# octaviogarcia/RaytracingOneWeekend

Hardware: AMD Instinct MI355X
Metric: Msamples/s (W×H×spp/s) + achieved HBM GB/s, 1080p@512spp traced scene (higher is better)
Workload: dtype f32; 1 GPU; C1 S-traced 1920x1080, 10496 spp timed (128 spp/step), depth 50; width=1920, height=1080, max_depth=50, parallelism=tile1, gather=RCCL send/recv (om_gather_frame), rccl_library=/usr/local/lib/python3.10/dist-packages/torch/lib/librccl.so, kernel=auto, pipeline=auto, tail_bounce=default, streams=2

## Files before the change

include/ottomarcher.h:

```cpp
#ifndef OTTOMARCHER_H
#define OTTOMARCHER_H

#include <stdint.h>
#include <stddef.h>

#ifdef __cplusplus
extern "C" {
#endif

#define OM_ABI_VERSION 2

typedef int32_t om_status;
#define OM_OK 0
#define OM_ERR_INVALID (-1)
#define OM_ERR_DEVICE (-2)
#define OM_ERR_STATE (-3)
#define OM_ERR_UNSUPPORTED (-4)
#define OM_ERR_NOMEM (-5)

enum { OM_LAMBERTIAN = 0, OM_METAL = 1, OM_DIELECTRIC = 2 };
typedef struct om_material {
    float albedo[3];
    float fuzz;
    float ior;
// ... 147 lines not shown
om_status om_occluded_rays(om_ctx* ctx, const om_query_params* q, const om_ray* rays,
                           const om_ray_window* windows, uint32_t n, uint8_t* occluded);
om_status om_hit_rays_windows_device(om_ctx* ctx, const om_query_params* q, const om_ray* dev_rays,
                                     const om_ray_window* dev_windows, uint32_t n, om_hit* dev_hits, void* stream);
om_status om_hit_rays_windows(om_ctx* ctx, const om_query_params* q, const om_ray* rays,
                              const om_ray_window* windows, uint32_t n, om_hit* hits);
#define OM_QUERY_BLOCK 512
uint32_t om_query_max_grid(om_ctx* ctx);
om_status om_host_register(void* p, size_t bytes);
om_status om_host_unregister(void* p);
om_status om_render_device(om_ctx* ctx, const om_camera* cam, const om_render_params* p, om_pixel_stats* dev_stats,
                           void* stream);
om_status om_render_device_pixels(om_ctx* ctx, const om_camera* cam, const om_render_params* p, om_pixel_stats* dev_stats,
                                  const uint32_t* dev_pixels, uint32_t n_pixels, void* stream);
om_status om_get_counters(om_ctx* ctx, om_counters* out);
om_status om_reset_counters(om_ctx* ctx, void* stream);
const volatile uint64_t* om_progress(om_ctx* ctx);
om_status om_reset_progress(om_ctx* ctx);
om_status om_set_counting(om_ctx* ctx, int32_t enable);
enum { OM_PIPELINE_MEGAKERNEL = 0, OM_PIPELINE_WAVEFRONT = 1, OM_PIPELINE_AUTO = 2 };
om_status om_set_pipeline(om_ctx* ctx, int32_t pipeline);
om_status om_set_tail_bounce(om_ctx* ctx, uint32_t bounce);

om_status om_set_streams(om_ctx* ctx, uint32_t streams);

om_status om_set_adaptive_batches(om_ctx* ctx, uint32_t batches, uint32_t paths_log2);

enum { OM_PRIMARY_LISTS_OFF = 0, OM_PRIMARY_LISTS_AUTO = 1, OM_PRIMARY_LISTS_ON = 2 };
om_status om_set_primary_lists(om_ctx* ctx, int32_t mode);

enum {
    OM_KT_BOUNCE0 = 0,
    OM_KT_BOUNCE = 1,
    OM_KT_TAIL = 2,
    OM_KT_ACCUMULATE = 3,
    OM_KT_MEGAKERNEL = 4,
    OM_KT_BOUNCE_SPAN = 5,
    OM_KT_N = 6
};
typedef struct om_kernel_times {
    uint64_t launches[OM_KT_N];
    double ms[OM_KT_N];
} om_kernel_times;
om_status om_set_timing(om_ctx* ctx, int32_t mode);
om_status om_get_kernel_times(om_ctx* ctx, om_kernel_times* out);

// ... 57 lines not shown
```

raytracingoneweekend_amd/_lib.py:

```python
import ctypes as C
import os

import numpy as np

_HERE = os.path.dirname(os.path.abspath(__file__))
LIB_PATH = os.environ.get("OM_LIB") or os.path.join(_HERE, "libottomarcher.so")

OM_OK = 0
OM_ERR_INVALID, OM_ERR_DEVICE, OM_ERR_STATE, OM_ERR_UNSUPPORTED, OM_ERR_NOMEM = -1, -2, -3, -4, -5
OM_LAMBERTIAN, OM_METAL, OM_DIELECTRIC = 0, 1, 2
OM_KERNEL_AUTO, OM_KERNEL_BRUTE, OM_KERNEL_CULLED, OM_KERNEL_BVH, OM_KERNEL_SBVH, OM_KERNEL_BVH2, OM_KERNEL_BVH4 = \
    0, 1, 2, 3, 4, 5, 6
OM_KERNEL_BVH2W = 7
KERNELS = {"auto": OM_KERNEL_AUTO, "brute": OM_KERNEL_BRUTE, "culled": OM_KERNEL_CULLED, "bvh": OM_KERNEL_BVH,
           "sbvh": OM_KERNEL_SBVH, "bvh2": OM_KERNEL_BVH2, "bvh4": OM_KERNEL_BVH4, "bvh2w": OM_KERNEL_BVH2W}
TREE_REGIMES = ("none", "lds", "l2", "wide", "fallback_bvh")
OM_PIPELINE_MEGAKERNEL, OM_PIPELINE_WAVEFRONT, OM_PIPELINE_AUTO = 0, 1, 2
PIPELINES = {"megakernel": OM_PIPELINE_MEGAKERNEL, "wavefront": OM_PIPELINE_WAVEFRONT, "auto": OM_PIPELINE_AUTO}

F3 = C.c_float * 3
F16 = C.c_float * 16


class om_material(C.Structure):
# ... 65 lines not shown
KT_CLASSES = ("bounce0", "bounce", "tail", "accumulate", "megakernel", "bounce_span")
VIEWS = ("normal", "samples", "sample_blur", "depth", "depth_blur", "ids", "id_blur")


class om_kernel_times(C.Structure):
    _fields_ = [("launches", C.c_uint64 * 6), ("ms", C.c_double * 6)]


PIXEL_STATS_DTYPE = np.dtype([("bloom", "<u8"), ("sum", "<f4", (3,)), ("n", "<u4"), ("avg_depth", "<f4"),
                              ("bad_avgs", "<u4"), ("color", "u1", (3,)), ("flags", "u1"), ("reserved", "<u4")])
assert PIXEL_STATS_DTYPE.itemsize == 40

EXPORTS = [
    "om_abi_version", "om_build_id", "om_material_lambertian", "om_material_metal", "om_material_metal_fuzz", "om_material_dielectric",
    "om_mat4_identity", "om_mat4_translate", "om_mat4_scale", "om_mat4_rotate", "om_mat4_mul",
    "om_mat4_fast_homogenous_inverse", "om_camera_new", "om_world_create", "om_world_destroy", "om_world_clear",
    "om_world_add_sphere", "om_world_add_sphere_radius", "om_world_add_cube", "om_world_add_cube_length",
    "om_world_add_triangle", "om_world_add_parallelogram", "om_world_add_triangle_basis",
    "om_world_add_parallelogram_basis", "om_world_add_plane", "om_world_add_marched_sphere",
    "om_world_add_marched_box", "om_world_add_marched_torus", "om_world_add_marched_sdf", "om_world_marched_sdf_count", "om_world_counts", "om_world_export",
    "om_world_random_scene", "om_world_basic_scene", "om_world_marched_scene", "om_create", "om_destroy",
    "om_last_error", "om_upload_world", "om_set_kernel", "om_render", "om_render_device",
    "om_render_device_pixels", "om_get_counters", "om_reset_counters", "om_set_counting", "om_set_pipeline",
    "om_set_tail_bounce", "om_set_streams", "om_set_adaptive_batches", "om_set_timing", "om_get_kernel_times", "om_display_device", "om_display",
    "om_write_bmp", "om_write_ppm", "om_set_primary_lists",
    "om_shard_capacity", "om_shard_pixels", "om_shard_assemble_host", "om_comm_unique_id", "om_comm_init_rank",
    "om_comm_destroy", "om_comm_info", "om_render_shard", "om_gather_frame", "om_scatter_frame", "om_multi_create",
    "om_multi_destroy", "om_multi_transport", "om_multi_ctx", "om_multi_upload_world", "om_multi_render",
    "om_multi_last_error", "om_progress", "om_reset_progress", "om_host_register", "om_host_unregister",
    "om_multi_render_host", "om_multi_gather", "om_multi_reset", "om_rccl_library",
    "om_hit_rays_device", "om_hit_rays", "om_world_object_material", "om_query_max_grid",
    "om_occluded_rays_device", "om_occluded_rays", "om_hit_rays_windows_device", "om_hit_rays_windows",
    "om_world_add_triangles", "om_world_tree_info", "om_get_tree_info",
]
OM_COMM_ID_BYTES = 128
OM_TRANSPORT_RCCL, OM_TRANSPORT_LOCAL = 0, 1


class OmError(RuntimeError):
    pass


def _share_hip_runtime_with_torch():
    try:
        import torch
    except Exception:
        pass
# ... 40 lines not shown
        "om_world_add_marched_sphere": (st, [vp, fp, C.c_float, mp]),
        "om_world_add_marched_box": (st, [vp, fp, fp, mp]),
        "om_world_add_marched_torus": (st, [vp, fp, fp, mp]),
        "om_world_add_marched_sdf": (st, [vp, fp, vp, C.c_uint32, mp]),
        "om_world_marched_sdf_count": (st, [vp, C.POINTER(C.c_uint32)]),
        "om_world_counts": (st, [vp, C.POINTER(C.c_uint32)]),
        "om_world_export": (st, [vp, C.c_int32, C.c_uint32, fp, C.c_uint32]),
        "om_world_random_scene": (st, [vp, C.c_uint64, C.c_uint32, C.c_int32]),
        "om_world_basic_scene": (st, [vp]),
        "om_world_marched_scene": (st, [vp]),
        "om_create": (st, [C.c_int32, C.POINTER(vp)]),
        "om_destroy": (None, [vp]),
        "om_last_error": (C.c_char_p, [vp]),
        "om_upload_world": (st, [vp, vp]),
        "om_set_kernel": (st, [vp, C.c_int32]),
        "om_render": (st, [vp, C.POINTER(om_camera), C.POINTER(om_render_params), vp, C.POINTER(om_counters)]),
        "om_render_device": (st, [vp, C.POINTER(om_camera), C.POINTER(om_render_params), vp, vp]),
        "om_render_device_pixels": (st, [vp, C.POINTER(om_camera), C.POINTER(om_render_params), vp, vp, C.c_uint32, vp]),
        "om_get_counters": (st, [vp, C.POINTER(om_counters)]),
        "om_reset_counters": (st, [vp, vp]),
        "om_set_counting": (st, [vp, C.c_int32]),
        "om_set_pipeline": (st, [vp, C.c_int32]),
        "om_set_tail_bounce": (st, [vp, C.c_uint32]),
        "om_set_streams": (st, [vp, C.c_uint32]),
        "om_set_adaptive_batches": (st, [vp, C.c_uint32, C.c_uint32]),
        "om_set_timing": (st, [vp, C.c_int32]),
        "om_get_kernel_times": (st, [vp, C.POINTER(om_kernel_times)]),
        "om_display_device": (st, [vp, vp, C.c_uint32, C.c_uint32, C.c_int32, vp, vp]),
        "om_display": (st, [vp, vp, C.c_uint32, C.c_uint32, C.c_int32, vp]),
        "om_write_bmp": (st, [C.c_char_p, vp, C.c_uint32, C.c_uint32]),
        "om_write_ppm": (st, [C.c_char_p, vp, C.c_uint32, C.c_uint32]),
        "om_set_primary_lists": (st, [vp, C.c_int32]),
        "om_shard_capacity": (C.c_uint32, [C.c_uint32, C.c_uint32, C.c_uint32]),
        "om_shard_pixels": (st, [C.c_uint32, C.c_uint32, C.c_uint32, C.c_uint32, vp, C.c_uint32, C.POINTER(C.c_uint32)]),
        "om_shard_assemble_host": (st, [C.c_uint32, C.c_uint32, C.c_uint32, C.POINTER(vp), vp]),
        "om_comm_unique_id": (st, [vp]),
        "om_comm_init_rank": (st, [vp, C.c_uint32, C.c_uint32, vp, C.POINTER(vp)]),
        "om_comm_destroy": (None, [vp]),
        "om_render_shard": (st, [vp, C.POINTER(om_camera), C.POINTER(om_render_params), vp, vp]),
        "om_gather_frame": (st, [vp, vp, C.c_uint32, C.c_uint32, vp, vp]),
        "om_scatter_frame": (st, [vp, vp, C.c_uint32, C.c_uint32, vp, vp]),
        "om_multi_create": (st, [C.POINTER(C.c_int32), C.c_uint32, C.POINTER(vp)]),
        "om_multi_destroy": (None, [vp]),
        "om_multi_transport": (C.c_int32, [vp]),
        "om_multi_ctx": (vp, [vp, C.c_uint32]),
        "om_multi_upload_world": (st, [vp, vp]),
# ... 59 lines not shown
```

raytracingoneweekend_amd/csrc/om_render.hip:

```cpp
#include <hip/hip_runtime.h>

#include <algorithm>
#include <cmath>
#include <cstring>
#include <mutex>
#include <new>
#include <string>
#include <vector>

#include "../../include/ottomarcher.h"
#include "om_device.h"
#include "om_layout.h"
#include "om_display.h"
#include "om_tiles.h"
#include "om_wavefront.h"
#include "om_world.h"
#include "om_internal.h"

using namespace omd;

static_assert(sizeof(om_pixel_stats) == 40, "om_pixel_stats layout");
static_assert(sizeof(om_ray) == 24 && sizeof(om_hit) == 32 && sizeof(om_query_params) == 16, "query record layouts");
static_assert(sizeof(om_ray_window) == 8, "query window layout");
static_assert(OM_QUERY_BLOCK == 512, "OM_QUERY_BLOCK is the wavefront workgroup size");
// ... 201 lines not shown
    void* p = nullptr;
    size_t n = 0;
    void release() { if (p) (void)hipFree(p); p = nullptr; n = 0; }
};

}

struct om_ctx {
    int device = 0;
    hipStream_t stream = nullptr;
    std::string err;
    std::vector<DevBuf> scene_bufs;
    OmSceneDev scene{};
    bool have_world = false;
    om_tree_info tree_info{};
    int kernel = OM_KERNEL_AUTO;
    DevBuf counters, stats, pixels, view_scratch, view_rgb;
    struct JitterTable { uint64_t seed; uint32_t spp; DevBuf buf; };
    std::vector<JitterTable> jitters;
    hipStream_t last_stream = nullptr;
    bool count_work = true;
    int pipeline = OM_PIPELINE_AUTO;
    uint32_t tail_bounce = 0;
    uint32_t wf_streams = 2;
    uint32_t ad_batches = 0, ad_paths_log2 = 0;
    std::vector<float> srec_box;
    uint64_t world_gen = 0;
    int primary_lists = OM_PRIMARY_LISTS_AUTO;
    DevBuf tile_off, tile_idx, tile_tnear;
    bool tiles_valid = false, tiles_use = false;
    om_camera tiles_cam{};
    uint32_t tiles_w = 0, tiles_h = 0;
    uint64_t tiles_gen = 0;
    double tiles_avg = 0.0;
    omw::Timer timer;
    omw::Buffers wf;
    unsigned long long* progress_host = nullptr;
    DevBuf frame_list;
    DevBuf query_rays, query_hits;
    DevBuf query_windows, query_occ;
    uint32_t frame_w = 0, frame_h = 0;
    ~om_ctx() {
        for (auto& b : scene_bufs) b.release();
        for (auto& j : jitters) j.buf.release();
        counters.release(); stats.release(); pixels.release(); frame_list.release();
        query_rays.release(); query_hits.release();
// ... 187 lines not shown
    P.progress = c->progress_host ? 1u : 0u;
    uint64_t threads;
    if (dev_pixels) {
        P.n_pixels = n_pixels;
        threads = n_pixels;
    } else {
        const uint64_t tiles = (uint64_t)P.tiles_x * ((p->height + 7u) / 8u);
        P.n_pixels = p->width * p->height;
        threads = tiles * 64u;
    }
    if (threads == 0) return OM_OK;
    int pipeline = c->pipeline;
    if (pipeline == OM_PIPELINE_AUTO) pipeline = OM_PIPELINE_WAVEFRONT;
    int mode = c->kernel;
    if (mode == OM_KERNEL_AUTO) mode = OM_KERNEL_BVH2;
    if (pipeline == OM_PIPELINE_WAVEFRONT) {
        omw::Launch L;
        L.S = c->scene; L.C = C; L.P = P;
        L.jitter = jitter;
        L.stats = dev_stats;
        L.counters = (unsigned long long*)c->counters.p;
        L.count = c->count_work;
        L.tail_bounce = c->tail_bounce;
        L.streams = c->wf_streams;
        L.ad_batches = c->ad_batches; L.ad_paths_log2 = c->ad_paths_log2;
        L.timer = &c->timer;
        L.tile_off = nullptr; L.tile_idx = nullptr; L.tile_tnear = nullptr;
        L.progress_host = c->progress_host;
        if ((mode == OM_KERNEL_BVH2 && c->scene.n_b2nodes) || (mode == OM_KERNEL_BVH2W && c->scene.n_b2wnodes)) {
            if ((s = ensure_tile_lists(c, cam, p->width, p->height, stream)) != OM_OK) return s;
            if (c->tiles_use) {
                L.tile_off = (const uint32_t*)c->tile_off.p; L.tile_idx = (const uint16_t*)c->tile_idx.p;
                L.tile_tnear = (const float*)c->tile_tnear.p;
            }
        }
        L.trace_mode = wf_trace_mode(mode);
        if (dev_pixels) {
            L.pixels = dev_pixels; L.n_pixels = n_pixels; L.stats_by_pixel = false;
        } else {
            if (c->frame_w != p->width || c->frame_h != p->height || !c->frame_list.p) {
                std::vector<uint32_t> lst;
                lst.reserve((size_t)p->width * p->height);
                const uint32_t tx = (p->width + 7u) / 8u, ty = (p->height + 7u) / 8u;
                for (uint32_t t = 0; t < tx * ty; ++t)
                    for (uint32_t l = 0; l < 64u; ++l) {
                        const uint32_t px = (t % tx) * 8u + (l & 7u), py = (t / tx) * 8u + (l >> 3);
// ... 308 lines not shown

om_status om_set_pipeline(om_ctx* c, int32_t pipeline) {
    if (!c) return set_err(nullptr, OM_ERR_INVALID, "null ctx");
    if (pipeline != OM_PIPELINE_MEGAKERNEL && pipeline != OM_PIPELINE_WAVEFRONT && pipeline != OM_PIPELINE_AUTO)
        return set_err(c, OM_ERR_INVALID, "om_set_pipeline: unknown pipeline");
    c->pipeline = pipeline;
    return OM_OK;
}

om_status om_set_primary_lists(om_ctx* c, int32_t mode) {
    if (!c) return set_err(nullptr, OM_ERR_INVALID, "null ctx");
    if (mode < OM_PRIMARY_LISTS_OFF || mode > OM_PRIMARY_LISTS_ON)
        return set_err(c, OM_ERR_INVALID, "om_set_primary_lists: unknown mode");
    c->primary_lists = mode;
    return OM_OK;
}

om_status om_set_tail_bounce(om_ctx* c, uint32_t bounce) {
    if (!c) return set_err(nullptr, OM_ERR_INVALID, "null ctx");
    c->tail_bounce = bounce;
    return OM_OK;
}

om_status om_set_streams(om_ctx* c, uint32_t streams) {
    if (!c) return set_err(nullptr, OM_ERR_INVALID, "null ctx");
    if (streams < 1 || streams > (uint32_t)omw::kMaxSets) return set_err(c, OM_ERR_INVALID, "om_set_streams: streams must be 1..4");
    c->wf_streams = streams;
    return OM_OK;
}

om_status om_set_adaptive_batches(om_ctx* c, uint32_t batches, uint32_t paths_log2) {
    if (!c) return set_err(nullptr, OM_ERR_INVALID, "null ctx");
    if (batches > 64u || paths_log2 > 27u)
        return set_err(c, OM_ERR_INVALID, "om_set_adaptive_batches: batches <= 64, paths_log2 <= 27");
    c->ad_batches = batches; c->ad_paths_log2 = paths_log2;
    return OM_OK;
}

om_status om_set_timing(om_ctx* c, int32_t mode) {
    if (!c) return set_err(nullptr, OM_ERR_INVALID, "null ctx");
    if (mode < 0 || mode > 2) return set_err(c, OM_ERR_INVALID, "om_set_timing: mode must be 0, 1 or 2");
    OM_HIP(c, hipSetDevice(c->device));
    for (size_t i = 0; c->timer.on() && i < c->timer.cls.size(); ++i)
        if (c->timer.cls[i] >= 0) OM_HIP(c, hipEventSynchronize(c->timer.ev[2 * i + 1]));
    c->timer.mode = mode;
    c->timer.clear();
// ... 120 lines not shown
```

raytracingoneweekend_amd/csrc/om_tuning.h:

```cpp
#pragma once

#ifndef OM_WF_BLOCK
#define OM_WF_BLOCK 512
#endif
#ifndef OM_WF_WAVES
#define OM_WF_WAVES 8
#endif
#ifndef OM_WF_TAIL_SPB
#define OM_WF_TAIL_SPB 2
#endif
#ifndef OM_WF_TAIL_WGS_PER_CU
#define OM_WF_TAIL_WGS_PER_CU 1
#endif
#ifndef OM_WF_MAX_PATHS_LOG2
#define OM_WF_MAX_PATHS_LOG2 27
#endif
#ifndef OM_WF_BATCH_SPP
#define OM_WF_BATCH_SPP 16
#endif
#ifndef OM_WF_MIN_PATHS_LOG2
#define OM_WF_MIN_PATHS_LOG2 25
#endif
#ifndef OM_WF_HYB_BYTES
#define OM_WF_HYB_BYTES 16384
#endif
#ifndef OM_WF_HYBW_BYTES
#define OM_WF_HYBW_BYTES 0
#endif
#ifndef OM_WF_HYB4_BYTES
#define OM_WF_HYB4_BYTES 0
#endif
#ifndef OM_WF_REFILL
#define OM_WF_REFILL 16
#endif
#ifndef OM_WF_TAIL_SHADE
// ... 45 lines not shown
```

raytracingoneweekend_amd/csrc/om_wavefront.h:

```cpp
#pragma once
#include <hip/hip_runtime.h>

#include <cstdint>
#include <string>
#include <vector>

#include "../../include/ottomarcher.h"
#include "om_layout.h"

namespace omw {

struct QueueSet {
    float4* q[2][3] = {{nullptr, nullptr, nullptr}, {nullptr, nullptr, nullptr}};
    uint4* qr[2] = {nullptr, nullptr};
    float4* res = nullptr;
    uint32_t* res_id = nullptr;
    uint32_t* counts = nullptr;
    float2* hit = nullptr;
    void release();
};

constexpr int kMaxSets = 4;
struct Buffers {
    uint64_t cap = 0;
    uint32_t counts_n = 0;
    int nsets = 0;
    QueueSet set[kMaxSets];
    uint32_t* n0 = nullptr;
    uint64_t n0_cap = 0;
    hipStream_t side[kMaxSets] = {};
    std::vector<hipEvent_t> ev;
    void release();
};
// ... 20 lines not shown
    void end(int i, int c, hipStream_t st, uint32_t launches = 1) {
        if (!on() || i < 0) return;
        (void)hipEventRecord(ev[2 * i + 1], st);
        cls[i] = c;
        nl[i] = launches;
    }
    void clear() { cls.clear(); nl.clear(); }
    void release() { for (auto e : ev) (void)hipEventDestroy(e); ev.clear(); clear(); }
};

struct Launch {
    OmSceneDev S;
    OmCamDev C;
    OmParamsDev P;
    const float2* jitter;
    om_pixel_stats* stats;
    const uint32_t* pixels;
    uint32_t n_pixels;
    bool stats_by_pixel;
    unsigned long long* counters;
    bool count;
    int trace_mode;
    uint32_t tail_bounce;
    uint32_t streams;
    uint32_t ad_batches;
    uint32_t ad_paths_log2;
    Timer* timer;
    const uint32_t* tile_off;
    const uint16_t* tile_idx;
    const float* tile_tnear;
    unsigned long long* progress_host;
};

hipError_t render(Buffers& B, const Launch& L, hipStream_t stream, std::string& err);

struct Query {
    OmSceneDev S;
    float tmin, tmax;
    uint32_t march_steps;
    const om_ray* rays;
    const om_ray_window* windows = nullptr;
    om_hit* hits = nullptr;
    uint8_t* occluded = nullptr;
    uint32_t n;
    unsigned long long* counters;
    bool count;
// ... 8 lines not shown
```

raytracingoneweekend_amd/csrc/om_wavefront.hip:

```cpp
#include "om_wavefront.h"

#include <algorithm>
#include <type_traits>

#include "om_device.h"
#include "om_trace.h"
#include "om_tuning.h"

using namespace omd;

namespace omw {

void QueueSet::release() {
    for (int a = 0; a < 2; ++a) {
        for (int b = 0; b < 3; ++b) { if (q[a][b]) (void)hipFree(q[a][b]); q[a][b] = nullptr; }
        if (qr[a]) (void)hipFree(qr[a]); qr[a] = nullptr;
    }
    if (res) (void)hipFree(res);
    if (res_id) (void)hipFree(res_id);
    if (counts) (void)hipFree(counts);
    if (hit) (void)hipFree(hit);
    res = nullptr; res_id = nullptr; counts = nullptr; hit = nullptr;
}

// ... 306 lines not shown
        s = (v & 0x7FFFFFFFu) + R.done + s_local;
        live = s < P.spp_total && !(v >> 31);
    } else {
        const om_pixel_stats& ps = R.stats[R.by_pixel ? pixel : k];
        s = ps.n + s_local;
        live = s < P.spp_total && !(P.adaptive && (ps.flags & 1u));
    }
    if (!live) {
        res_id[i] = kNoSample;
        return false;
    }
    p.g = path_rng(P.skey, pixel, s);
    const uint32_t line = pixel / P.width;
    gen_camera_ray(R.C, P, R.jitter, (float)(pixel - P.width * line), (float)line, s, p.g, p.o, p.d);
    p.cur = f3(1.0f, 1.0f, 1.0f); p.depthf = 0.0f; p.first_id = 0u; p.seg = 0u; p.slot = (uint32_t)i;
    return true;
}

template <int TR, bool COUNT, bool MARCH, bool FIRST, bool HIT = false, bool USER = MARCH>
__global__ __launch_bounds__(kBlk) OM_WAVES_ATTR void k_bounce(OmSceneDev S, OmParamsDev P, Seg G, Gen R, Queue in,
                                                 const uint32_t* __restrict__ count_in, Queue out,
                                                 uint32_t* __restrict__ count_out, float4* __restrict__ res,
                                                 uint32_t* __restrict__ res_id, unsigned long long* __restrict__ counters,
                                                 const float2* __restrict__ hitbuf, uint32_t* __restrict__ tail_next) {
    const uint64_t seg0 = (uint64_t)blockIdx.x * G.segcap;
    uint32_t n, stride = R.n_pixels;
    uint64_t first0 = seg0;
    if (FIRST) {
        if (tail_next && blockIdx.x == 0 && threadIdx.x == 0) *tail_next = 0u;
        uint64_t paths = (uint64_t)R.n_pixels * R.batch;
        if (R.ad.list) {
            const AdPlan pl = uniform_load(R.ad.plan);
            stride = pl.c;
            paths = (uint64_t)pl.c * ad_batch(pl.c, pl.done, R.ad.j, R.ad.A);
            first0 = (uint64_t)blockIdx.x * seg_capacity(paths, G.nseg);
            n = first0 < paths ? (uint32_t)std::min<uint64_t>(seg_capacity(paths, G.nseg), paths - first0) : 0u;
        } else {
            n = seg0 < paths ? (uint32_t)std::min<uint64_t>(G.segcap, paths - seg0) : 0u;
        }
    } else {
        n = count_in[blockIdx.x];
    }
    if (n == 0) {
        if (threadIdx.x == 0) count_out[blockIdx.x] = 0u;
        return;
    }
    __shared__ uint32_t q_next, q_out;
    if (threadIdx.x == 0) { q_next = kBlk / 64u; q_out = 0u; }
    __syncthreads();
    const Tracer T = HIT ? Tracer{} : stage_scene<TR>(S);
    const uint32_t depth_cap = P.max_depth > 1u ? P.max_depth : 1u;
    WorkT<COUNT, false, tr_bary(TR)> w;
    uint32_t segs = 0;
    const uint32_t lane = __lane_id();
    for (uint32_t chunk = __builtin_amdgcn_readfirstlane(threadIdx.x >> 6); chunk * 64u < n;) {
        const uint32_t jj = chunk * 64u + lane;
        bool keep = false;
        Path p;
        uint32_t p_pixel = 0;
        if (jj < n) {
            const uint64_t i = seg0 + jj;
            bool live = true;
            if (FIRST) {
                live = gen_path(P, R, stride, first0 + jj, p, p_pixel, res_id);
            } else {
                load_ray(in, i, p);
                load_rest(in, i, p);
            }
            if (live) {
                float closest;
                int best;
                if (HIT) {
                    const float2 h = hitbuf[i];
                    closest = h.x; best = __float_as_int(h.y);
                } else if (FIRST && (tr_base(TR) == TR_BVH2_LDS || tr_base(TR) == TR_BVH2_GLOBAL || tr_base(TR) == TR_BVH2_WIDE) && R.tile_off) {
                    const uint32_t line = p_pixel / P.width;
                    const uint32_t tile = (p_pixel - line * P.width) / 8u + (line / 8u) * P.tiles_x;
                    closest = P.tmax;
                    const uint32_t t0 = __builtin_amdgcn_readfirstlane(tile);
                    if (__ballot(tile != t0) == 0)
                        best = traced_tiles<true>(S, R.tile_off, R.tile_idx, t0, p.o, p.d, P.tmin, closest, w, R.tile_tnear);
                    else
                        best = traced_tiles(S, R.tile_off, R.tile_idx, tile, p.o, p.d, P.tmin, closest, w);
                    if (MARCH) {
                        float tm;
                        const int mg = march(S, p.o, p.d, P.tmin, P.tmax, closest, P.march_steps, tm, w);
                        if (mg >= 0) { best = mg; closest = tm; }
                    }
                } else {
                    best = trace<TR, MARCH>(S, P, T, p.o, p.d, closest, w);
                }
                keep = shade_path<MARCH, USER>(S, P, depth_cap, p, closest, best, res, res_id);
                if (COUNT) segs++;
            }
        }
        const uint64_t m = __ballot(keep);
        uint32_t obase = 0u, nc = 0u;
        if (lane == 0) {
            obase = m ? atomicAdd(&q_out, (uint32_t)__popcll(m)) : 0u;
            nc = atomicAdd(&q_next, 1u);
        }
        obase = __builtin_amdgcn_readfirstlane(obase);
        chunk = __builtin_amdgcn_readfirstlane(nc);
        if (keep) store_path(out, seg0 + obase + (uint32_t)__popcll(m & ((1ull << lane) - 1ull)), p);
    }
    __syncthreads();
    if (threadIdx.x == 0) count_out[blockIdx.x] = q_out;
    if (COUNT) {
        flush_counter(counters, OMC_SEGMENTS, segs);
        flush_counter(counters, OMC_PRIM_TESTS, w.prim);
        flush_counter(counters, OMC_PRE_TESTS, w.pre);
        flush_counter(counters, OMC_MARCH, w.march);
    }
}

template <bool COUNT>
__global__ __launch_bounds__(kBlk) OM_WAVES_ATTR void k_raygen(OmParamsDev P, Seg G, Gen R, Queue out,
                                                 uint32_t* __restrict__ count_out, uint32_t* __restrict__ res_id) {
    const uint64_t seg0 = (uint64_t)blockIdx.x * G.segcap;
    uint64_t paths = (uint64_t)R.n_pixels * R.batch, first0 = seg0;
    uint32_t n, stride = R.n_pixels;
    if (R.ad.list) {
        const AdPlan pl = uniform_load(R.ad.plan);
        stride = pl.c;
        paths = (uint64_t)pl.c * ad_batch(pl.c, pl.done, R.ad.j, R.ad.A);
        first0 = (uint64_t)blockIdx.x * seg_capacity(paths, G.nseg);
        n = first0 < paths ? (uint32_t)std::min<uint64_t>(seg_capacity(paths, G.nseg), paths - first0) : 0u;
    } else {
        n = seg0 < paths ? (uint32_t)std::min<uint64_t>(G.segcap, paths - seg0) : 0u;
    }
// ... 68 lines not shown
                                                const uint32_t* __restrict__ count_in, float2* __restrict__ hit,
                                                unsigned long long* __restrict__ counters) {
    const uint32_t n = count_in[blockIdx.x];
    if (n == 0) return;
    const uint64_t seg0 = (uint64_t)blockIdx.x * G.segcap;
    __shared__ uint32_t next;
    if (threadIdx.x == 0) next = kBlk;
    __syncthreads();
    const Tracer T = stage_scene<TR>(S);
    WorkT<COUNT, false, tr_bary(TR)> w;
    if constexpr (VIEW == MV_EXACT_C2_LDS) {
        __shared__ MarchedC2Lds::Block mblock;
        march_lanes<TR, COUNT>(S, P, T, MarchedC2Lds(S, &mblock), in, seg0, n, next, hit, w);
    } else {
        march_lanes<TR, COUNT>(S, P, T, MarchedArrays(S), in, seg0, n, next, hit, w);
    }
    if (COUNT) {
        flush_counter(counters, OMC_PRIM_TESTS, w.prim);
        flush_counter(counters, OMC_PRE_TESTS, w.pre);
        flush_counter(counters, OMC_MARCH, w.march);
    }
}

struct TailSrc {
    const Queue& in;
    const uint32_t* pre;
    uint32_t s0, ns, segcap;
    __device__ __forceinline__ bool load(uint32_t idx, Path& p) const {
        uint32_t lo = 0, hi = ns;
        while (hi - lo > 1u) {
            const uint32_t mid = (lo + hi) >> 1;
            if (pre[mid] <= idx) lo = mid; else hi = mid;
        }
        const uint64_t i = (uint64_t)(s0 + lo) * segcap + (idx - pre[lo]);
        load_ray(in, i, p);
        load_rest(in, i, p);
        return true;
    }
};
template <int TR, bool COUNT, class M, class Src, class Wk>
__device__ __forceinline__ uint32_t tail_march_lanes(const OmSceneDev& S, const OmParamsDev& P, const Tracer& T, const M& m,
                                                     const Src& src, uint32_t total, uint32_t& next,
                                                     float4* __restrict__ res, uint32_t* __restrict__ res_id, Wk& w) {
    const uint32_t lane = __lane_id();
    const uint32_t depth_cap = P.max_depth > 1u ? P.max_depth : 1u;
    uint32_t idx = threadIdx.x, segs = 0, iters = 0;
    bool have = idx < total, dry = !have, marching = false, act = false;
    __shared__ uint32_t rest[9][kBlk];
    Path p;
    float t = 0.0f, closest = 0.0f;
    int best = -1;
    auto park = [&]() {
        const uint32_t i = threadIdx.x;
        rest[0][i] = __float_as_uint(p.cur.x); rest[1][i] = __float_as_uint(p.cur.y); rest[2][i] = __float_as_uint(p.cur.z);
        rest[3][i] = __float_as_uint(p.depthf); rest[4][i] = p.first_id; rest[5][i] = p.seg; rest[6][i] = p.slot;
        rest[7][i] = p.g.s; rest[8][i] = p.g.k;
    };
// ... 47 lines not shown
}

template <int TR, bool COUNT, int VIEW = MV_ARRAYS, uint32_t SPB = kTailSpb>
__global__ __launch_bounds__(kBlk) __attribute__((amdgpu_waves_per_eu(OM_WF_TAIL_MARCH_WAVES, OM_WF_TAIL_MARCH_WAVES)))
void k_tail_march(OmSceneDev S, OmParamsDev P, Seg G, Queue in,
                                               const uint32_t* __restrict__ count_in, float4* __restrict__ res,
                                               uint32_t* __restrict__ res_id, unsigned long long* __restrict__ counters) {
    __shared__ uint32_t pre[SPB + 1];
    __shared__ uint32_t next;
    const uint32_t s0 = blockIdx.x * SPB;
    if (threadIdx.x == 0) {
        uint32_t acc = 0;
        for (uint32_t k = 0; k < SPB; ++k) {
            pre[k] = acc;
            acc += s0 + k < G.nseg ? count_in[s0 + k] : 0u;
        }
        pre[SPB] = acc;
        next = kBlk;
    }
    __syncthreads();
    const uint32_t total = pre[SPB];
    if (total == 0) return;
    const Tracer T = stage_scene<TR>(S);
    const TailSrc src{in, pre, s0, SPB, G.segcap};
    WorkT<COUNT, false, tr_bary(TR)> w;
    uint32_t segs = 0;
    if constexpr (VIEW == MV_EXACT_C2_LDS) {
        __shared__ MarchedC2Lds::Block mblock;
        segs = tail_march_lanes<TR, COUNT>(S, P, T, MarchedC2Lds(S, &mblock), src, total, next, res, res_id, w);
    } else {
        segs = tail_march_lanes<TR, COUNT>(S, P, T, MarchedArrays(S), src, total, next, res, res_id, w);
    }
    if (COUNT) {
        flush_counter(counters, OMC_SEGMENTS, segs);
        flush_counter(counters, OMC_PRIM_TESTS, w.prim);
        flush_counter(counters, OMC_PRE_TESTS, w.pre);
        flush_counter(counters, OMC_MARCH, w.march);
    }
}

template <int TR, bool COUNT>
__global__ __launch_bounds__(kBlk) OM_WAVES_ATTR
void k_tail(OmSceneDev S, OmParamsDev P, Seg G, Queue in, const uint32_t* __restrict__ count_in, uint32_t pre_off,
            uint32_t* __restrict__ next, float4* __restrict__ res, uint32_t* __restrict__ res_id,
            unsigned long long* __restrict__ counters) {
    uint32_t* pre = (uint32_t*)wf_lds + pre_off / 4u;
    __shared__ uint32_t wave_sum[kWaves];
    const uint32_t lane = __lane_id(), wave = threadIdx.x >> 6;
    const uint32_t per = (G.nseg + kBlk - 1u) / kBlk;
    const uint32_t c0 = threadIdx.x * per, c1 = c0 + per < G.nseg ? c0 + per : G.nseg;
    uint32_t mine = 0;
    for (uint32_t k = c0; k < c1; ++k) mine += count_in[k];
    uint32_t incl = mine;
#pragma unroll
    for (int off = 1; off < 64; off <<= 1) {
        const uint32_t v = __shfl_up(incl, off, 64);
        if (lane >= (uint32_t)off) incl += v;
    }
    if (lane == 63u) wave_sum[wave] = incl;
    __syncthreads();
    uint32_t acc = incl - mine, total = 0;
#pragma unroll
    for (uint32_t k = 0; k < kWaves; ++k) {
        const uint32_t v = wave_sum[k];
        if (k < wave) acc += v;
        total += v;
    }
    if (total == 0) return;
    for (uint32_t k = c0; k < c1; ++k) { pre[k] = acc; acc += count_in[k]; }
    if (threadIdx.x == 0) pre[G.nseg] = total;
    __syncthreads();
    const Tracer T = stage_scene<TR>(S);
    const uint32_t depth_cap = P.max_depth > 1u ? P.max_depth : 1u;
    const TailSrc src{in, pre, 0u, G.nseg, G.segcap};
    WorkT<COUNT, false, tr_bary(TR)> w;
    uint32_t segs = 0;
    const uint32_t lanes = gridDim.x * kBlk;
    const uint32_t round = (wave + kWaves - blockIdx.x % kWaves) % kWaves;
    uint32_t idx = (round * gridDim.x + blockIdx.x) * 64u + lane;
    bool have = idx < total;
    bool more = total > lanes;
    Path p;
    if (have) src.load(idx, p);
    for (;;) {
        if (have) {
            float closest;
            const int best = trace<TR, false>(S, P, T, p.o, p.d, closest, w);
            if (COUNT) segs++;
            have = shade_path<false>(S, P, depth_cap, p, closest, best, res, res_id);
        }
        if (more) {
            const uint64_t want = __ballot(!have);
            if (want) {
                const uint32_t nw = (uint32_t)__popcll(want);
                uint32_t base = 0u;
                if (lane == 0) base = atomicAdd(next, nw);
                base = lanes + __builtin_amdgcn_readfirstlane(base);
// ... 289 lines not shown
            QueueSet& S = B.set[k];
            if (S.counts) (void)hipFree(S.counts);
            S.counts = nullptr;
            if ((e = hipMalloc(&S.counts, (size_t)counts_n * sizeof(uint32_t))) != hipSuccess) return e;
        }
        B.counts_n = counts_n;
    }
    return hipSuccess;
}

Queue queue(QueueSet& B, int k) { return Queue{B.q[k][0], B.q[k][1], B.q[k][2], B.qr[k]}; }

inline uint32_t tail_pre_off(uint32_t lds) { return (lds + 15u) & ~15u; }
inline uint32_t tail_lds(uint32_t lds, uint32_t nseg) { return tail_pre_off(lds) + (nseg + 1u) * 4u; }

template <int TR, bool COUNT, bool MARCH>
uint32_t run_batch(QueueSet& B, const Launch& L, hipStream_t st, Seg G, const Gen& R, uint32_t depth_cap,
                   uint32_t tail_at, uint32_t lds, uint32_t tail_grid) {
    Timer& tm = *L.timer;
    const bool each = tm.mode == 1;
    uint32_t launches = 0;
    const bool exact = MARCH && L.S.n_msdf == 0u && MarchedC2Lds::matches(L.S.n_msph, L.S.n_mbox, L.S.n_mtor);
    uint32_t* const tail_next = B.counts + (size_t)(depth_cap + 1u) * G.nseg;
    auto tail = [&](const Queue& in, const uint32_t* cin) {
        const int ti = each ? tm.begin(st) : -1;
        if constexpr (MARCH) {
            const uint32_t grid = (G.nseg + kTailSpb - 1u) / kTailSpb;
            if (exact && exact_view_built<TR>())
                hipLaunchKernelGGL((k_tail_march<TR, COUNT, exact_view_built<TR>() ? MV_EXACT_C2_LDS : MV_ARRAYS>), dim3(grid),
                                   dim3(kBlk), lds, st, L.S, L.P, G, in, cin, B.res, B.res_id, L.counters);
            else
                hipLaunchKernelGGL((k_tail_march<TR, COUNT>), dim3(grid), dim3(kBlk), lds, st, L.S, L.P, G, in, cin,
                                   B.res, B.res_id, L.counters);
        } else {
            hipLaunchKernelGGL((k_tail<TR, COUNT>), dim3(tail_grid), dim3(kBlk), tail_lds(lds, G.nseg), st, L.S, L.P, G, in, cin,
                               tail_pre_off(lds), tail_next, B.res, B.res_id, L.counters);
        }
        tm.end(ti, OM_KT_TAIL, st);
        return launches + 1u;
    };
    if constexpr (MARCH) {
        {
            const int ti = each ? tm.begin(st) : -1;
            hipLaunchKernelGGL((k_raygen<COUNT>), dim3(G.nseg), dim3(kBlk), 0, st, L.P, G, R, queue(B, 0), B.counts, B.res_id);
            tm.end(ti, OM_KT_BOUNCE0, st);
            ++launches;
        }
        for (uint32_t bounce = 0; bounce < depth_cap; ++bounce) {
            const Queue in = queue(B, bounce & 1u), out = queue(B, (bounce + 1u) & 1u);
            const uint32_t* cin = B.counts + (size_t)bounce * G.nseg;
            if (bounce >= tail_at) return tail(in, cin);
            uint32_t* cout = B.counts + (size_t)(bounce + 1u) * G.nseg;
            const int kc = bounce == 0 ? OM_KT_BOUNCE0 : OM_KT_BOUNCE;
            int ti = each ? tm.begin(st) : -1;
            if (exact && exact_view_built<TR>())
                hipLaunchKernelGGL((k_march<TR, COUNT, exact_view_built<TR>() ? MV_EXACT_C2_LDS : MV_ARRAYS>), dim3(G.nseg),
                                   dim3(kBlk), lds, st, L.S, L.P, G, in, cin, B.hit, L.counters);
            else
                hipLaunchKernelGGL((k_march<TR, COUNT, MV_ARRAYS>), dim3(G.nseg), dim3(kBlk), lds, st, L.S, L.P, G, in, cin,
                                   B.hit, L.counters);
            tm.end(ti, kc, st);
            ti = each ? tm.begin(st) : -1;
            if (exact && exact_view_built<TR>())
                hipLaunchKernelGGL((k_bounce<TR, COUNT, MARCH, false, true, false>), dim3(G.nseg), dim3(kBlk), 0, st, L.S, L.P, G,
                                   R, in, cin, out, cout, B.res, B.res_id, L.counters, (const float2*)B.hit, (uint32_t*)nullptr);
            else
                hipLaunchKernelGGL((k_bounce<TR, COUNT, MARCH, false, true>), dim3(G.nseg), dim3(kBlk), 0, st, L.S, L.P, G, R, in,
                                   cin, out, cout, B.res, B.res_id, L.counters, (const float2*)B.hit, (uint32_t*)nullptr);
            tm.end(ti, kc, st);
            launches += 2u;
        }
        return launches;
    } else {
    for (uint32_t bounce = 0; bounce < depth_cap; ++bounce) {
        const Queue in = queue(B, bounce & 1u), out = queue(B, (bounce + 1u) & 1u);
        const uint32_t* cin = B.counts + (size_t)bounce * G.nseg;
        if (bounce > 0 && bounce >= tail_at) return tail(in, cin);
        uint32_t* cout = B.counts + (size_t)(bounce + 1u) * G.nseg;
        const int ti = each ? tm.begin(st) : -1;
        if (bounce == 0)
            hipLaunchKernelGGL((k_bounce<TR, COUNT, MARCH, true>), dim3(G.nseg), dim3(kBlk), lds, st, L.S, L.P, G, R, in,
                               cin, out, cout, B.res, B.res_id, L.counters, (const float2*)nullptr, tail_next);
        else
            hipLaunchKernelGGL((k_bounce<TR, COUNT, MARCH, false>), dim3(G.nseg), dim3(kBlk), lds, st, L.S, L.P, G, R, in,
                               cin, out, cout, B.res, B.res_id, L.counters, (const float2*)nullptr, (uint32_t*)nullptr);
        tm.end(ti, bounce == 0 ? OM_KT_BOUNCE0 : OM_KT_BOUNCE, st);
        ++launches;
    }
    return launches;
    }
}

template <int TR>
uint32_t run_tr(bool count, bool march, QueueSet& B, const Launch& L, hipStream_t st, Seg G, const Gen& R,
                uint32_t depth_cap, uint32_t tail_at, uint32_t lds, uint32_t tail_grid) {
    if (count && march) return run_batch<TR, true, true>(B, L, st, G, R, depth_cap, tail_at, lds, tail_grid);
    if (count) return run_batch<TR, true, false>(B, L, st, G, R, depth_cap, tail_at, lds, tail_grid);
    if (march) return run_batch<TR, false, true>(B, L, st, G, R, depth_cap, tail_at, lds, tail_grid);
    return run_batch<TR, false, false>(B, L, st, G, R, depth_cap, tail_at, lds, tail_grid);
}

hipError_t ensure_events(Buffers& B, size_t n) {
    while (B.ev.size() < n) {
        hipEvent_t e = nullptr;
        const hipError_t r = hipEventCreateWithFlags(&e, hipEventDisableTiming);
        if (r != hipSuccess) return r;
        B.ev.push_back(e);
    }
// ... 98 lines not shown
        if (concurrent) batch = std::min<uint32_t>(batch, (L.P.sample_count + want - 1u) / want);
        while (done_at.back() < L.P.sample_count)
            done_at.push_back(done_at.back() + std::min(batch, L.P.sample_count - done_at.back()));
        nb = (uint32_t)done_at.size() - 1u;
        ns = concurrent ? std::min<uint32_t>(want, nb) : 1u;
        max_paths = (uint64_t)n_px * batch;
    }
    const uint32_t depth_cap = L.P.max_depth > 1u ? L.P.max_depth : 1u;
    int dev = 0;
    (void)hipGetDevice(&dev);
    int cus = 256;
    (void)hipDeviceGetAttribute(&cus, hipDeviceAttributeMultiprocessorCount, dev);
    const int tr = pick_trace(L.trace_mode, L.S);
    const bool march = (L.S.n_msph + L.S.n_mbox + L.S.n_mtor + L.S.n_msdf) != 0u;
    const bool l2_tree = tr_base(tr) == TR_BVH2_GLOBAL || tr_base(tr) == TR_BVH4_GLOBAL || tr_base(tr) == TR_BVH2_WIDE;
    const uint32_t tail_at = L.tail_bounce ? L.tail_bounce
                           : march ? kTailMarched : l2_tree ? kTailL2
                           : adaptive ? OM_WF_ADAPTIVE_TAIL
                           : max_paths > (1ull << 25) ? kTailBigBatch : kTailDefault;
    const uint32_t lanes_per_cu = (march || l2_tree) ? OM_WF_LANES_PER_CU_WIDE : OM_WF_LANES_PER_CU;
    uint32_t nseg = (uint32_t)std::min<uint64_t>((max_paths + kBlk - 1) / kBlk, (uint64_t)cus * (lanes_per_cu / kBlk));
    nseg = (nseg + kTailSpb - 1) / kTailSpb * kTailSpb;
    const uint32_t segcap = seg_capacity(max_paths, nseg);
    hipError_t e = grow(B, (uint64_t)nseg * segcap, (depth_cap + 1u) * nseg + 1u, (int)ns);
    if (e != hipSuccess) { err = "wavefront buffer allocation failed"; return e; }
    const uint32_t lds = trace_lds(tr, L.S);
    const uint32_t tail_grid = (uint32_t)cus * kTailWgsPerCu;
    int lds_max = 0;
    (void)hipDeviceGetAttribute(&lds_max, hipDeviceAttributeMaxSharedMemoryPerBlock, dev);
    if (!march && tail_at < depth_cap && tail_lds(lds, nseg) > (uint32_t)lds_max) {
        err = "the tail's LDS request exceeds the device's limit";
        return hipErrorInvalidValue;
    }
    if (lds > (uint32_t)lds_max) {
        err = "the traversal's LDS request exceeds the device's limit";
        return hipErrorInvalidValue;
    }
    Gen R;
    R.C = L.C; R.jitter = L.jitter; R.stats = L.stats; R.pixels = L.pixels; R.n_pixels = n_px;
    R.by_pixel = L.stats_by_pixel ? 1u : 0u;
    R.tile_off = L.tile_off; R.tile_idx = L.tile_idx; R.tile_tnear = L.tile_tnear;
    R.n0 = nullptr; R.done = 0; R.ad = AdList{};
    hipStream_t streams[kMaxSets] = {st, st, st, st};
    Timer& tm = *L.timer;
    const int call_ti = tm.begin(st);
    const uint32_t plan_stride = ad_k + 1u;
    const uint64_t words = adaptive ? (uint64_t)ns * 2u * cmax + (uint64_t)ns * plan_stride * 2u : (ns > 1 ? n_px : 0u);
// ... 127 lines not shown
```

Measured before the change: 7311 Msamples/s.

## Split wavefront path queue by ray direction into front and back regions

Surviving paths in each bounce kernel are partitioned by direction: rays with d.y at or below a threshold are written from the top end of each segment and the rest from the bottom, with a separate per-segment count. The next bounce and the tail kernel remap indices so that the two groups are processed as contiguous runs. The aim is more coherent traversal inside a wavefront (sky-bound rays versus ground-bound rays), reducing divergence and improving cache locality. It costs an extra ballot, an extra atomic per wave, doubled count buffers and index remapping on every load.

```diff
diff --git a/include/ottomarcher.h b/include/ottomarcher.h
--- a/include/ottomarcher.h
+++ b/include/ottomarcher.h
@@ -193,6 +193,8 @@
 om_status om_set_pipeline(om_ctx* ctx, int32_t pipeline);
 om_status om_set_tail_bounce(om_ctx* ctx, uint32_t bounce);
 
+om_status om_set_queue_split(om_ctx* ctx, int32_t mode);
+
 om_status om_set_streams(om_ctx* ctx, uint32_t streams);
 
 om_status om_set_adaptive_batches(om_ctx* ctx, uint32_t batches, uint32_t paths_log2);
diff --git a/raytracingoneweekend_amd/_lib.py b/raytracingoneweekend_amd/_lib.py
--- a/raytracingoneweekend_amd/_lib.py
+++ b/raytracingoneweekend_amd/_lib.py
@@ -111,7 +111,7 @@
     "om_world_random_scene", "om_world_basic_scene", "om_world_marched_scene", "om_create", "om_destroy",
     "om_last_error", "om_upload_world", "om_set_kernel", "om_render", "om_render_device",
     "om_render_device_pixels", "om_get_counters", "om_reset_counters", "om_set_counting", "om_set_pipeline",
-    "om_set_tail_bounce", "om_set_streams", "om_set_adaptive_batches", "om_set_timing", "om_get_kernel_times", "om_display_device", "om_display",
+    "om_set_tail_bounce", "om_set_queue_split", "om_set_streams", "om_set_adaptive_batches", "om_set_timing", "om_get_kernel_times", "om_display_device", "om_display",
     "om_write_bmp", "om_write_ppm", "om_set_primary_lists",
     "om_shard_capacity", "om_shard_pixels", "om_shard_assemble_host", "om_comm_unique_id", "om_comm_init_rank",
     "om_comm_destroy", "om_comm_info", "om_render_shard", "om_gather_frame", "om_scatter_frame", "om_multi_create",
@@ -198,6 +198,7 @@
         "om_set_counting": (st, [vp, C.c_int32]),
         "om_set_pipeline": (st, [vp, C.c_int32]),
         "om_set_tail_bounce": (st, [vp, C.c_uint32]),
+        "om_set_queue_split": (st, [vp, C.c_int32]),
         "om_set_streams": (st, [vp, C.c_uint32]),
         "om_set_adaptive_batches": (st, [vp, C.c_uint32, C.c_uint32]),
         "om_set_timing": (st, [vp, C.c_int32]),
diff --git a/raytracingoneweekend_amd/csrc/om_render.hip b/raytracingoneweekend_amd/csrc/om_render.hip
--- a/raytracingoneweekend_amd/csrc/om_render.hip
+++ b/raytracingoneweekend_amd/csrc/om_render.hip
@@ -247,6 +247,7 @@
     bool count_work = true;
     int pipeline = OM_PIPELINE_AUTO;
     uint32_t tail_bounce = 0;
+    uint32_t queue_split = 1;
     uint32_t wf_streams = 2;
     uint32_t ad_batches = 0, ad_paths_log2 = 0;
     std::vector<float> srec_box;
@@ -480,6 +481,7 @@
         L.counters = (unsigned long long*)c->counters.p;
         L.count = c->count_work;
         L.tail_bounce = c->tail_bounce;
+        L.queue_split = c->queue_split;
         L.streams = c->wf_streams;
         L.ad_batches = c->ad_batches; L.ad_paths_log2 = c->ad_paths_log2;
         L.timer = &c->timer;
@@ -834,6 +836,13 @@
     return OM_OK;
 }
 
+om_status om_set_queue_split(om_ctx* c, int32_t mode) {
+    if (!c) return set_err(nullptr, OM_ERR_INVALID, "null ctx");
+    if (mode != 0 && mode != 1) return set_err(c, OM_ERR_INVALID, "om_set_queue_split: mode must be 0 or 1");
+    c->queue_split = (uint32_t)mode;
+    return OM_OK;
+}
+
 om_status om_set_streams(om_ctx* c, uint32_t streams) {
     if (!c) return set_err(nullptr, OM_ERR_INVALID, "null ctx");
     if (streams < 1 || streams > (uint32_t)omw::kMaxSets) return set_err(c, OM_ERR_INVALID, "om_set_streams: streams must be 1..4");
diff --git a/raytracingoneweekend_amd/csrc/om_tuning.h b/raytracingoneweekend_amd/csrc/om_tuning.h
--- a/raytracingoneweekend_amd/csrc/om_tuning.h
+++ b/raytracingoneweekend_amd/csrc/om_tuning.h
@@ -11,6 +11,9 @@
 #endif
 #ifndef OM_WF_TAIL_WGS_PER_CU
 #define OM_WF_TAIL_WGS_PER_CU 1
+#endif
+#ifndef OM_WF_SPLIT_DY
+#define OM_WF_SPLIT_DY 0.3f
 #endif
 #ifndef OM_WF_MAX_PATHS_LOG2
 #define OM_WF_MAX_PATHS_LOG2 27
diff --git a/raytracingoneweekend_amd/csrc/om_wavefront.h b/raytracingoneweekend_amd/csrc/om_wavefront.h
--- a/raytracingoneweekend_amd/csrc/om_wavefront.h
+++ b/raytracingoneweekend_amd/csrc/om_wavefront.h
@@ -9,6 +9,10 @@
 #include "om_layout.h"
 
 namespace omw {
+
+__host__ __device__ inline uint32_t split_slot(uint32_t j, uint32_t nB, uint32_t segcap) {
+    return j < nB ? segcap - nB + j : j - nB;
+}
 
 struct QueueSet {
     float4* q[2][3] = {{nullptr, nullptr, nullptr}, {nullptr, nullptr, nullptr}};
@@ -75,6 +79,7 @@
     bool count;
     int trace_mode;
     uint32_t tail_bounce;
+    uint32_t queue_split;
     uint32_t streams;
     uint32_t ad_batches;
     uint32_t ad_paths_log2;
diff --git a/raytracingoneweekend_amd/csrc/om_wavefront.hip b/raytracingoneweekend_amd/csrc/om_wavefront.hip
--- a/raytracingoneweekend_amd/csrc/om_wavefront.hip
+++ b/raytracingoneweekend_amd/csrc/om_wavefront.hip
@@ -352,7 +352,10 @@
                                                  const uint32_t* __restrict__ count_in, Queue out,
                                                  uint32_t* __restrict__ count_out, float4* __restrict__ res,
                                                  uint32_t* __restrict__ res_id, unsigned long long* __restrict__ counters,
-                                                 const float2* __restrict__ hitbuf, uint32_t* __restrict__ tail_next) {
+                                                 const float2* __restrict__ hitbuf, uint32_t* __restrict__ tail_next,
+                                                 const uint32_t* __restrict__ count_in_b, uint32_t* __restrict__ count_out_b,
+                                                 uint32_t split) {
+    constexpr bool SPLIT = !MARCH && !HIT;
     const uint64_t seg0 = (uint64_t)blockIdx.x * G.segcap;
     uint32_t n, stride = R.n_pixels;
     uint64_t first0 = seg0;
@@ -372,11 +375,15 @@
         n = count_in[blockIdx.x];
     }
     if (n == 0) {
-        if (threadIdx.x == 0) count_out[blockIdx.x] = 0u;
+        if (threadIdx.x == 0) {
+            count_out[blockIdx.x] = 0u;
+            if (SPLIT) count_out_b[blockIdx.x] = 0u;
+        }
         return;
     }
-    __shared__ uint32_t q_next, q_out;
-    if (threadIdx.x == 0) { q_next = kBlk / 64u; q_out = 0u; }
+    const uint32_t nb_in = SPLIT && !FIRST ? count_in_b[blockIdx.x] : 0u;
+    __shared__ uint32_t q_next, q_out, q_out_b;
+    if (threadIdx.x == 0) { q_next = kBlk / 64u; q_out = 0u; q_out_b = 0u; }
     __syncthreads();
     const Tracer T = HIT ? Tracer{} : stage_scene<TR>(S);
     const uint32_t depth_cap = P.max_depth > 1u ? P.max_depth : 1u;
@@ -389,7 +396,7 @@
         Path p;
         uint32_t p_pixel = 0;
         if (jj < n) {
-            const uint64_t i = seg0 + jj;
+            const uint64_t i = seg0 + (SPLIT ? omw::split_slot(jj, nb_in, G.segcap) : jj);
             bool live = true;
             if (FIRST) {
                 live = gen_path(P, R, stride, first0 + jj, p, p_pixel, res_id);
@@ -424,18 +431,30 @@
                 if (COUNT) segs++;
             }
         }
-        const uint64_t m = __ballot(keep);
-        uint32_t obase = 0u, nc = 0u;
+        const bool back = SPLIT && keep && split != 0u && !(p.d.y > OM_WF_SPLIT_DY);
+        const uint64_t mb = SPLIT ? __ballot(back) : 0ull;
+        const uint64_t m = __ballot(keep) & ~mb;
+        uint32_t obase = 0u, obase_b = 0u, nc = 0u;
         if (lane == 0) {
             obase = m ? atomicAdd(&q_out, (uint32_t)__popcll(m)) : 0u;
+            if (SPLIT) obase_b = mb ? atomicAdd(&q_out_b, (uint32_t)__popcll(mb)) : 0u;
             nc = atomicAdd(&q_next, 1u);
         }
         obase = __builtin_amdgcn_readfirstlane(obase);
+        if (SPLIT) obase_b = __builtin_amdgcn_readfirstlane(obase_b);
         chunk = __builtin_amdgcn_readfirstlane(nc);
-        if (keep) store_path(out, seg0 + obase + (uint32_t)__popcll(m & ((1ull << lane) - 1ull)), p);
+        if (keep) {
+            const uint64_t below = (1ull << lane) - 1ull;
+            const uint32_t slot = back ? G.segcap - 1u - (obase_b + (uint32_t)__popcll(mb & below))
+                                       : obase + (uint32_t)__popcll(m & below);
+            store_path(out, seg0 + slot, p);
+        }
     }
     __syncthreads();
-    if (threadIdx.x == 0) count_out[blockIdx.x] = q_out;
+    if (threadIdx.x == 0) {
+        count_out[blockIdx.x] = q_out + q_out_b;
+        if (SPLIT) count_out_b[blockIdx.x] = q_out_b;
+    }
     if (COUNT) {
         flush_counter(counters, OMC_SEGMENTS, segs);
         flush_counter(counters, OMC_PRIM_TESTS, w.prim);
@@ -550,17 +569,20 @@
     }
 }
 
+template <bool SPLIT>
 struct TailSrc {
     const Queue& in;
     const uint32_t* pre;
     uint32_t s0, ns, segcap;
+    const uint32_t* nb;
     __device__ __forceinline__ bool load(uint32_t idx, Path& p) const {
         uint32_t lo = 0, hi = ns;
         while (hi - lo > 1u) {
             const uint32_t mid = (lo + hi) >> 1;
             if (pre[mid] <= idx) lo = mid; else hi = mid;
         }
-        const uint64_t i = (uint64_t)(s0 + lo) * segcap + (idx - pre[lo]);
+        const uint32_t j = idx - pre[lo];
+        const uint64_t i = (uint64_t)(s0 + lo) * segcap + (SPLIT ? omw::split_slot(j, nb[s0 + lo], segcap) : j);
         load_ray(in, i, p);
         load_rest(in, i, p);
         return true;
@@ -654,7 +676,7 @@
     const uint32_t total = pre[SPB];
     if (total == 0) return;
     const Tracer T = stage_scene<TR>(S);
-    const TailSrc src{in, pre, s0, SPB, G.segcap};
+    const TailSrc<false> src{in, pre, s0, SPB, G.segcap, nullptr};
     WorkT<COUNT, false, tr_bary(TR)> w;
     uint32_t segs = 0;
     if constexpr (VIEW == MV_EXACT_C2_LDS) {
@@ -673,7 +695,8 @@
 
 template <int TR, bool COUNT>
 __global__ __launch_bounds__(kBlk) OM_WAVES_ATTR
-void k_tail(OmSceneDev S, OmParamsDev P, Seg G, Queue in, const uint32_t* __restrict__ count_in, uint32_t pre_off,
+void k_tail(OmSceneDev S, OmParamsDev P, Seg G, Queue in, const uint32_t* __restrict__ count_in,
+            const uint32_t* __restrict__ count_in_b, uint32_t pre_off,
             uint32_t* __restrict__ next, float4* __restrict__ res, uint32_t* __restrict__ res_id,
             unsigned long long* __restrict__ counters) {
     uint32_t* pre = (uint32_t*)wf_lds + pre_off / 4u;
@@ -704,7 +727,7 @@
     __syncthreads();
     const Tracer T = stage_scene<TR>(S);
     const uint32_t depth_cap = P.max_depth > 1u ? P.max_depth : 1u;
-    const TailSrc src{in, pre, 0u, G.nseg, G.segcap};
+    const TailSrc<true> src{in, pre, 0u, G.nseg, G.segcap, count_in_b};
     WorkT<COUNT, false, tr_bary(TR)> w;
     uint32_t segs = 0;
     const uint32_t lanes = gridDim.x * kBlk;
@@ -1040,7 +1063,8 @@
     uint32_t launches = 0;
     const bool exact = MARCH && L.S.n_msdf == 0u && MarchedC2Lds::matches(L.S.n_msph, L.S.n_mbox, L.S.n_mtor);
     uint32_t* const tail_next = B.counts + (size_t)(depth_cap + 1u) * G.nseg;
-    auto tail = [&](const Queue& in, const uint32_t* cin) {
+    uint32_t* const counts_b = tail_next + 1;
+    auto tail = [&](const Queue& in, const uint32_t* cin, const uint32_t* cinb) {
         const int ti = each ? tm.begin(st) : -1;
         if constexpr (MARCH) {
             const uint32_t grid = (G.nseg + kTailSpb - 1u) / kTailSpb;
@@ -1052,7 +1076,7 @@
                                    B.res, B.res_id, L.counters);
         } else {
             hipLaunchKernelGGL((k_tail<TR, COUNT>), dim3(tail_grid), dim3(kBlk), tail_lds(lds, G.nseg), st, L.S, L.P, G, in, cin,
-                               tail_pre_off(lds), tail_next, B.res, B.res_id, L.counters);
+                               cinb, tail_pre_off(lds), tail_next, B.res, B.res_id, L.counters);
         }
         tm.end(ti, OM_KT_TAIL, st);
         return launches + 1u;
@@ -1067,7 +1091,7 @@
         for (uint32_t bounce = 0; bounce < depth_cap; ++bounce) {
             const Queue in = queue(B, bounce & 1u), out = queue(B, (bounce + 1u) & 1u);
             const uint32_t* cin = B.counts + (size_t)bounce * G.nseg;
-            if (bounce >= tail_at) return tail(in, cin);
+            if (bounce >= tail_at) return tail(in, cin, nullptr);
             uint32_t* cout = B.counts + (size_t)(bounce + 1u) * G.nseg;
             const int kc = bounce == 0 ? OM_KT_BOUNCE0 : OM_KT_BOUNCE;
             int ti = each ? tm.begin(st) : -1;
@@ -1081,10 +1105,12 @@
             ti = each ? tm.begin(st) : -1;
             if (exact && exact_view_built<TR>())
                 hipLaunchKernelGGL((k_bounce<TR, COUNT, MARCH, false, true, false>), dim3(G.nseg), dim3(kBlk), 0, st, L.S, L.P, G,
-                                   R, in, cin, out, cout, B.res, B.res_id, L.counters, (const float2*)B.hit, (uint32_t*)nullptr);
+                                   R, in, cin, out, cout, B.res, B.res_id, L.counters, (const float2*)B.hit, (uint32_t*)nullptr,
+                                   (const uint32_t*)nullptr, (uint32_t*)nullptr, 0u);
             else
                 hipLaunchKernelGGL((k_bounce<TR, COUNT, MARCH, false, true>), dim3(G.nseg), dim3(kBlk), 0, st, L.S, L.P, G, R, in,
-                                   cin, out, cout, B.res, B.res_id, L.counters, (const float2*)B.hit, (uint32_t*)nullptr);
+                                   cin, out, cout, B.res, B.res_id, L.counters, (const float2*)B.hit, (uint32_t*)nullptr,
+                                   (const uint32_t*)nullptr, (uint32_t*)nullptr, 0u);
             tm.end(ti, kc, st);
             launches += 2u;
         }
@@ -1093,15 +1119,19 @@
     for (uint32_t bounce = 0; bounce < depth_cap; ++bounce) {
         const Queue in = queue(B, bounce & 1u), out = queue(B, (bounce + 1u) & 1u);
         const uint32_t* cin = B.counts + (size_t)bounce * G.nseg;
-        if (bounce > 0 && bounce >= tail_at) return tail(in, cin);
+        const uint32_t* cinb = counts_b + (size_t)bounce * G.nseg;
+        if (bounce > 0 && bounce >= tail_at) return tail(in, cin, cinb);
         uint32_t* cout = B.counts + (size_t)(bounce + 1u) * G.nseg;
+        uint32_t* coutb = counts_b + (size_t)(bounce + 1u) * G.nseg;
         const int ti = each ? tm.begin(st) : -1;
         if (bounce == 0)
             hipLaunchKernelGGL((k_bounce<TR, COUNT, MARCH, true>), dim3(G.nseg), dim3(kBlk), lds, st, L.S, L.P, G, R, in,
-                               cin, out, cout, B.res, B.res_id, L.counters, (const float2*)nullptr, tail_next);
+                               cin, out, cout, B.res, B.res_id, L.counters, (const float2*)nullptr, tail_next, cinb, coutb,
+                               L.queue_split);
         else
             hipLaunchKernelGGL((k_bounce<TR, COUNT, MARCH, false>), dim3(G.nseg), dim3(kBlk), lds, st, L.S, L.P, G, R, in,
-                               cin, out, cout, B.res, B.res_id, L.counters, (const float2*)nullptr, (uint32_t*)nullptr);
+                               cin, out, cout, B.res, B.res_id, L.counters, (const float2*)nullptr, (uint32_t*)nullptr, cinb,
+                               coutb, L.queue_split);
         tm.end(ti, bounce == 0 ? OM_KT_BOUNCE0 : OM_KT_BOUNCE, st);
         ++launches;
     }
@@ -1246,7 +1276,7 @@
     uint32_t nseg = (uint32_t)std::min<uint64_t>((max_paths + kBlk - 1) / kBlk, (uint64_t)cus * (lanes_per_cu / kBlk));
     nseg = (nseg + kTailSpb - 1) / kTailSpb * kTailSpb;
     const uint32_t segcap = seg_capacity(max_paths, nseg);
-    hipError_t e = grow(B, (uint64_t)nseg * segcap, (depth_cap + 1u) * nseg + 1u, (int)ns);
+    hipError_t e = grow(B, (uint64_t)nseg * segcap, 2u * (depth_cap + 1u) * nseg + 1u, (int)ns);
     if (e != hipSuccess) { err = "wavefront buffer allocation failed"; return e; }
     const uint32_t lds = trace_lds(tr, L.S);
     const uint32_t tail_grid = (uint32_t)cus * kTailWgsPerCu;
```

Result: no change. 7358 Msamples/s (median of 6 runs) (+0.6%).
